# Quyans/GOI-Hyperplane

Measured on AMD Instinct MI355X. Metric: training views/sec (rasterizer fwd+bwd), 1M Gaussians @1600x1056 RGB+16-d feat, higher is better.
Workload: dtype f32

## Files before the change

### goi_hyperplane_amd/_lib.py

```python
from __future__ import annotations

import ctypes as C
import os

_HERE = os.path.dirname(os.path.abspath(__file__))
LIB_PATH = os.path.join(_HERE, "lib", "libgoi_raster.so")

ABI_VERSION = 8

STAGES = ("preprocess", "depth_sort", "scan", "emit", "tile_sort", "ranges", "blend_fwd", "blend_bwd",
          "preprocess_bwd")


class GoiRasterScene(C.Structure):
    _fields_ = [
        ("P", C.c_int), ("D", C.c_int), ("M", C.c_int), ("S", C.c_int), ("W", C.c_int), ("H", C.c_int),
        ("bg", C.c_void_p), ("means3D", C.c_void_p), ("shs", C.c_void_p), ("colors_precomp", C.c_void_p),
        ("semantics", C.c_void_p), ("opacities", C.c_void_p), ("scales", C.c_void_p),
        ("scale_modifier", C.c_float), ("rotations", C.c_void_p), ("cov3D_precomp", C.c_void_p),
        ("viewmatrix", C.c_void_p), ("projmatrix", C.c_void_p), ("campos", C.c_void_p),
        ("tan_fovx", C.c_float), ("tan_fovy", C.c_float), ("prefiltered", C.c_int), ("debug", C.c_int),
    ]


# ... 83 lines not shown
    "goi_raster_photometric_backward": (C.c_int, [C.c_void_p, C.c_void_p, C.c_longlong, C.c_int, C.c_int, C.c_int, C.c_int, C.c_float,
                                           C.c_uint] + [C.c_void_p] * 5),
    "goi_raster_densify_workspace_bytes": (C.c_size_t, [C.c_longlong]),
    "goi_raster_densify_stats": (C.c_int, [C.c_longlong, C.c_void_p, C.c_longlong] + [C.c_void_p] * 4),
    "goi_raster_densify_plan": (C.c_int, [C.c_longlong] + [C.c_void_p] * 4 + [C.c_double] * 3 + [C.c_int, C.c_double, C.c_double]
                                + [C.c_void_p] * 3),
    "goi_raster_densify_prune_plan": (C.c_int, [C.c_longlong] + [C.c_void_p] * 4),
    "goi_raster_densify_apply": (C.c_int, [C.c_longlong, C.c_void_p, C.c_int] + [C.c_void_p] * 3 + [C.c_longlong, C.c_longlong]
                                 + [C.c_void_p] * 2),
    "goi_raster_set_option": (C.c_int, [C.c_char_p, C.c_int]),
    "goi_raster_blend_stats": (C.c_int, [C.c_int] * 4 + [C.c_void_p] * 5),
    "goi_raster_debug_views": (C.c_int, [C.c_int] * 4 + [C.c_void_p] * 3 + [C.c_void_p] * 8 + [C.c_void_p]),
    "goi_raster_debug_sort_workspace_bytes": (C.c_size_t, [C.c_longlong, C.c_int, C.c_int]),
    "goi_raster_debug_sort_pairs": (C.c_int, [C.c_void_p] * 4 + [C.c_longlong, C.c_int, C.c_int, C.c_void_p, C.c_void_p, C.c_int]
                                    + [C.c_void_p] * 3),
    "goi_raster_debug_scan_workspace_bytes": (C.c_size_t, [C.c_longlong]),
    "goi_raster_debug_exclusive_scan": (C.c_int, [C.c_void_p] * 3 + [C.c_longlong] + [C.c_void_p] * 4),
    "goi_raster_debug_reduce_row_floats": (C.c_int, [C.c_int, C.c_int]),
    "goi_raster_debug_reduce_workspace_bytes": (C.c_size_t, [C.c_longlong]),
    "goi_raster_debug_reduce_rows": (C.c_int, [C.c_int, C.c_int, C.c_int, C.c_longlong] + [C.c_void_p] * 14),
    "goi_raster_debug_preprocess_backward": (C.c_int, [C.POINTER(GoiRasterScene), C.c_int, C.c_int, C.c_int, C.c_longlong]
                                             + [C.c_void_p] * 22),
    "goi_raster_debug_pair_eval": (C.c_int, [C.c_int, C.c_int, C.c_int, C.c_void_p, C.c_void_p, C.c_longlong] + [C.c_void_p] * 4),
    "goi_raster_debug_backward_blend": (C.c_int, [C.POINTER(GoiRasterScene), C.c_int, C.c_int] + [C.c_void_p] * 24),
}

_lib = None


def load():
# ... 69 lines not shown
```

### goi_hyperplane_amd/csrc/api.hip

```cpp
#include <climits>
#include <cmath>
#include <cstdio>
#include <cstring>
#include <cstdlib>
#include <atomic>
#include <chrono>
#include <mutex>
#include <thread>
#include <string>
#include <vector>

#include "common.h"

namespace goi {

namespace {

thread_local std::string g_err;

int fail(const char* where, hipError_t e) {
    g_err = std::string(where) + ": " + hipGetErrorString(e);
    return -1;
}
int fail(const std::string& msg) {
// ... 224 lines not shown
    GOI_HIP(hipMemsetAsync(g.blk_coarse, 0,
                           round_up_256((size_t)(reinterpret_cast<char*>(g.scratch + depth_ctrl) -
                                                 reinterpret_cast<char*>(g.blk_coarse))), s));
    {
        StageTimer t(GOI_STAGE_PREPROCESS, s);
        launch_preprocess_fwd(sc, g, radii, im.ranges, gx * gy, s, zcut, zlearn, keep, keep_invert);
    }
    if (check_stage(sc, s, "preprocess")) return -1;
    if (ticket >= 0 && enqueue_readback(g, ticket, s)) return -1;
    const bool onesweep = g_options.sort_variant == 1;
    const uint32_t* v_dev = g.counters + COUNTER_V;
    int order_idx;
    {
        StageTimer t(GOI_STAGE_DEPTH_SORT, s);
        launch_compact_listed(P, g, onesweep ? radix_sort_ghist(g.scratch, (size_t)P, 0, 32) : nullptr, !onesweep, s);
        order_idx = radix_sort_pairs(g.sort_keys, g.sort_vals, (size_t)P, 0, 32, g.scratch, s, true,
                                     onesweep, onesweep ? v_dev : nullptr, g.counters + COUNTER_SORTERR);
    }
    if (check_stage(sc, s, "depth sort")) return -1;
    *order_out = g.sort_vals[order_idx];
    {
        StageTimer t(GOI_STAGE_SCAN, s);
        exclusive_scan_u32(g.tiles_touched, *order_out, g.offsets, (size_t)P, nullptr, g.scratch, s, v_dev);
    }
    return 0;
}

int enqueue_back(const GoiRasterScene& sc, GeomView& g, ImageView& im, const BinView& bv_in, int cap, bool exact,
                 const uint32_t* order, const int* radii, const uint32_t** plist, hipStream_t s) {
    BinView bv = bv_in;
    const int P = sc.P;
    const int gx = (sc.W + TILE - 1) / TILE, gy = (sc.H + TILE - 1) / TILE;
// ... 5 lines not shown
        if (counting) {
            launch_emit_counting(P, sc.W, sc.H, g, order, radii, bv.keys[0], bv.vals[0], im.ranges, bv.scratch,
                                 radix_sort_control_words((size_t)cap, 0, tile_bits), (uint32_t)cap, s);
        }
        else if (cap > 0)
            launch_emit(P, sc.W, sc.H, g, order, radii, bv.keys[0], bv.vals[0], (uint32_t)cap, s);
    }
    if (check_stage(sc, s, "emit")) return -1;
    int fin;
    if (counting) {
        {
            StageTimer t(GOI_STAGE_RANGES, s);
            launch_tile_ranges_hist(sc.W, sc.H, im.ranges, radix_sort_ghist(bv.scratch, (size_t)cap, 0, tile_bits), g.counters, s);
        }
        StageTimer t(GOI_STAGE_TILE_SORT, s);
        fin = radix_sort_pairs(bv.keys, bv.vals, (size_t)cap, 0, tile_bits, bv.scratch, s, true,
                               true, n_dev, g.counters + COUNTER_OVF);
    } else {
        {
            StageTimer t(GOI_STAGE_TILE_SORT, s);
            fin = radix_sort_pairs(bv.keys, bv.vals, (size_t)cap, 0, tile_bits, bv.scratch, s, false, false, n_dev,
                                   g.counters + COUNTER_OVF);
        }
        if (check_stage(sc, s, "tile sort")) return -1;
        StageTimer t(GOI_STAGE_RANGES, s);
        launch_ranges(cap, n_dev, bv.keys[fin], im.ranges, gx * gy, s);
    }
    if (check_stage(sc, s, "tile sort / ranges")) return -1;
    *plist = bv.vals[fin];
    return 0;
}

// ... 980 lines not shown
int goi_raster_set_option(const char* name, int value) {
    if (!name) return fail("option name is NULL");
    std::lock_guard<std::mutex> lk(g_options_mu);
    Options& g_options = g_shared_options;
    if (!strcmp(name, "fwd_variant")) {
        if (value < 0 || value > 1) return fail("fwd_variant must be 0 or 1");
        g_options.fwd_variant = value;
    }
    else if (!strcmp(name, "bwd_variant")) {
        if (value < 0 || value > 2) return fail("bwd_variant must be 0, 1 or 2");
        g_options.bwd_variant = value;
    }
    else if (!strcmp(name, "sort_variant")) g_options.sort_variant = value;
    else if (!strcmp(name, "sort_small")) g_options.sort_small = value;
    else if (!strcmp(name, "sort_lookback")) g_options.sort_lookback = value;
    else if (!strcmp(name, "cull_variant")) g_options.cull_variant = value;
    else if (!strcmp(name, "bwd_order")) {
        if (value < 0 || value > 8) return fail("bwd_order must be 0 .. 8");
        g_options.bwd_order = value;
    }
    else if (!strcmp(name, "decode_variant")) g_options.decode_variant = value;
    else if (!strcmp(name, "bwd_masks")) {
        if (value < 0 || value > 1) return fail("bwd_masks must be 0 or 1");
        g_options.bwd_masks = value;
    }
    else if (!strcmp(name, "bwd_records")) {
        if (value < 0 || value > 2) return fail("bwd_records must be 0, 1 or 2");
        g_options.bwd_records = value;
    }
    else if (!strcmp(name, "bwd_skip_idle")) {
// ... 65 lines not shown
                                 hipMemcpyDeviceToDevice, s));
    }
    if (depths) GOI_HIP(hipMemcpy2DAsync(depths, 4, rec + 44, pitch, 4, P, hipMemcpyDeviceToDevice, s));
    if (rgb) GOI_HIP(hipMemcpy2DAsync(rgb, 12, rec + 32, pitch, 12, P, hipMemcpyDeviceToDevice, s));
    if (tiles_touched)
        GOI_HIP(hipMemcpyAsync(tiles_touched, g.tiles_touched, sizeof(uint32_t) * P, hipMemcpyDeviceToDevice, s));
    if (ranges) GOI_HIP(hipMemcpyAsync(ranges, im.ranges, sizeof(uint2) * gx * gy, hipMemcpyDeviceToDevice, s));
    if (n_contrib)
        GOI_HIP(hipMemcpyAsync(n_contrib, im.n_contrib, sizeof(uint32_t) * (size_t)W * H, hipMemcpyDeviceToDevice, s));
    if (point_list && R > 0) {
        BinView bv;
        binning_layout(R, const_cast<char*>(static_cast<const char*>(binning_buffer)), &bv);
        const int fin = tile_sort_result_index(W, H, R);
        GOI_HIP(hipMemcpyAsync(point_list, bv.vals[fin], sizeof(uint32_t) * (size_t)R, hipMemcpyDeviceToDevice, s));
    }
    return 0;
}

static int debug_sort_args(const char* fn, long long n, int lo, int hi) {
    if (n < 0 || n >= SORT_MAX_KEYS) return fail(std::string(fn) + ": need 0 <= n < 2^30");
    if (lo < 0 || hi > 32 || lo >= hi) return fail(std::string(fn) + ": need 0 <= lo < hi <= 32");
    return 0;
}

size_t goi_raster_debug_sort_workspace_bytes(long long n, int lo, int hi) {
    if (n < 0 || n >= SORT_MAX_KEYS || lo < 0 || hi > 32 || lo >= hi) return 0;
    return sort_scratch_words((size_t)(n > 0 ? n : 1)) * sizeof(uint32_t) + 256;
}

int goi_raster_debug_sort_pairs(uint32_t* keys0, uint32_t* vals0, uint32_t* keys1, uint32_t* vals1, long long n, int lo, int hi,
// ... 11 lines not shown
    const hipStream_t s = static_cast<hipStream_t>(stream);
    uint32_t* scratch = static_cast<uint32_t*>(workspace);
    bool cleared = (flags & 1) != 0;
    if (ghist) {
        const size_t passes = (size_t)(hi - lo + 7) / 8;
        GOI_HIP(hipMemsetAsync(scratch, 0, radix_sort_control_words((size_t)n, lo, hi) * sizeof(uint32_t), s));
        GOI_HIP(hipMemcpyAsync(radix_sort_ghist(scratch, (size_t)n, lo, hi), ghist, passes * 256 * sizeof(uint32_t),
                               hipMemcpyDeviceToDevice, s));
        cleared = true;
    }
    uint32_t* keys[2] = {keys0, keys1};
    uint32_t* vals[2] = {vals0, vals1};
    const int fin = radix_sort_pairs(keys, vals, (size_t)n, lo, hi, scratch, s, cleared, ghist != nullptr, n_dev, error_out);
    GOI_HIP(hipGetLastError());
    if (error_out) radix_sort_report_error(scratch, (size_t)n, lo, hi, error_out, s);
    GOI_HIP(hipGetLastError());
    return fin;
}

size_t goi_raster_debug_scan_workspace_bytes(long long n) {
    return (n >= 0 && n < (1ll << 32)) ? scan_scratch_words((size_t)n) * sizeof(uint32_t) + 256 : 0;
}

int goi_raster_debug_exclusive_scan(const uint32_t* in, const uint32_t* gather, uint32_t* out, long long n, const uint32_t* n_dev,
                                    uint32_t* total, void* workspace, void* stream) {
    refresh_options();
    if (n < 0 || n >= (1ll << 32)) return fail("goi_raster_debug_exclusive_scan: need 0 <= n < 2^32");
    if (gather && out == in) return fail("goi_raster_debug_exclusive_scan: out == in with a gather is a data race");
    const hipStream_t s = static_cast<hipStream_t>(stream);
    if (n > 0 && (!in || !out || !workspace)) return fail("goi_raster_debug_exclusive_scan: a required pointer is NULL");
// ... 251 lines not shown
```

### goi_hyperplane_amd/csrc/common.h

```cpp
#pragma once

#include <hip/hip_runtime.h>
#include <stddef.h>
#include <stdint.h>

#include "goi_raster.h"

namespace goi {

constexpr int TILE = 16;
constexpr int TILE_PIX = TILE * TILE;
constexpr int WAVE = 64;

struct GaussRec {
    float4 q0, q1, q2;
};

struct GeomView {
    GaussRec* rec;
    float* cov3D;
    uint32_t* tiles_touched;
    uint8_t* clamped;
    uint32_t* sort_keys[2];
    uint32_t* sort_vals[2];
// ... 47 lines not shown

__host__ __device__ inline unsigned long long* member_mask_ptr(unsigned long long* qmask0, unsigned long long* qmask, int tile,
                                                                int q, uint32_t x0, int r) {
    return r == 0 ? qmask0 + ((size_t)tile * 4 + q) : qmask + (((size_t)(x0 >> 6) + (size_t)r) * 4 + q);
}

size_t geom_layout(int P, char* base, GeomView* v);
size_t image_layout(int W, int H, char* base, ImageView* v);
size_t binning_layout(int N, char* base, BinView* v);

struct Options {
    int fwd_variant = 1;
    int bwd_variant = 0;
    int sort_variant = 1;
    int sort_lookback = 1;
    int sort_small = 0;
    int decode_variant = 1;
    int cull_variant = 2;
    int bwd_order = 1;
    int bwd_masks = 1;
    int bwd_records = 1;
    int bwd_skip_idle = 1;
    int osh_path = 0;
};
extern thread_local Options g_options;
void refresh_options();

size_t scan_scratch_words(size_t n);
size_t sort_scratch_words(size_t n);
void exclusive_scan_u32(const uint32_t* in, const uint32_t* gather, uint32_t* out, size_t n, uint32_t* total,
                        uint32_t* scratch, hipStream_t s, const uint32_t* n_dev = nullptr);
int radix_sort_pairs(uint32_t* keys[2], uint32_t* vals[2], size_t n, int lo, int hi, uint32_t* scratch,
                     hipStream_t s, bool cleared = false, bool ghist_ready = false, const uint32_t* n_dev = nullptr,
                     uint32_t* frame_error = nullptr);
size_t radix_sort_control_words(size_t n, int lo, int hi);
uint32_t* radix_sort_ghist(uint32_t* scratch, size_t n, int lo, int hi);
void radix_sort_report_error(const uint32_t* scratch, size_t n, int lo, int hi, uint32_t* out, hipStream_t s);
constexpr long long SORT_MAX_KEYS = 1ll << 30;

void launch_preprocess_fwd(const GoiRasterScene& sc, const GeomView& g, int* radii, uint2* ranges, int n_tiles,
                           hipStream_t s, const float* zcut = nullptr, uint32_t* zlearn = nullptr,
                           const uint8_t* keep = nullptr, int keep_invert = 0);
void launch_compact_listed(int P, const GeomView& g, uint32_t* ghist, bool pad, hipStream_t s);
constexpr int COARSE_BLOCKS = 32, COARSE_STRIDE = 8;
constexpr int SORT_MAX_PASSES = 4, SORT_GH_COPIES = 8;
constexpr int PRE_BLOCK = 256;
void launch_emit(int P, int W, int H, const GeomView& g, const uint32_t* order, const int* radii, uint32_t* keys,
                 uint32_t* vals, uint32_t cap, hipStream_t s);
bool emit_can_count_tiles(int W, int H);
// ... 179 lines not shown
constexpr int NR_STRIPES = 32, NR_STRIDE = 32, NR_BASE = 32;
constexpr int COUNTER_WORDS = NR_BASE + NR_STRIPES * NR_STRIDE;
constexpr int COUNTER_CULL = 2;
constexpr int COUNTER_N = 3;
constexpr int COUNTER_V = 5;
constexpr int COUNTER_OVF = 4;

constexpr uint32_t OVF_TRUNCATED = 1u, OVF_MISSORTED = 2u, OVF_CUT_TOO_TIGHT = 4u;
constexpr int COUNTER_BIGQ = 7;
constexpr int COUNTER_SORTERR = 6;

inline int depth_sort_result_index() { return ((32 + 7) / 8) & 1; }

inline int tile_key_bits(uint32_t n_tiles) { return n_tiles <= 1 ? 1 : 32 - __builtin_clz(n_tiles); }

}
```

### goi_hyperplane_amd/csrc/preprocess.hip

```cpp
#include <algorithm>
#include <type_traits>

#include "common.h"
#include "gmath.h"
#include "row_sum.h"

namespace goi {

namespace {

__device__ __forceinline__ float ndc_to_pix(float v, int S) { return (float)(((v + 1.0) * S - 1.0) * 0.5); }

__device__ __forceinline__ M3 rotation_from_quat(float r, float x, float y, float z) {
    return make_m3(1.f - 2.f * (y * y + z * z), 2.f * (x * y - r * z), 2.f * (x * z + r * y),
                   2.f * (x * y + r * z), 1.f - 2.f * (x * x + z * z), 2.f * (y * z - r * x),
                   2.f * (x * z - r * y), 2.f * (y * z + r * x), 1.f - 2.f * (x * x + y * y));
}

struct Cov2D {
    M3 T, Vrk, W;
    V3 t;
    float txtz, tytz, limx, limy;
    M3 cov;
};
// ... 222 lines not shown
                    for (int i = 0; i < 8; i++) {
                        const int bsafe = max(bits[i], 0);
                        zc[i] = a.zcut[(size_t)(y0 + bsafe / w) * a.gx + (x0 + bsafe % w)];
                    }
#pragma unroll
                    for (int i = 0; i < 8; i++)
                        if (bits[i] >= 0 && zc[i] < p_view.z) mask &= ~(1ull << bits[i]);
                }
            }
            tmask_v = mask;
            touched = (uint32_t)__popcll(mask);
        }
        key = __float_as_uint(p_view.z);
    }

    if (vis) {
        float4* r4 = reinterpret_cast<float4*>(rec + idx);
        r4[0] = make_float4(pix, piy, con_a, con_b);
        r4[1] = make_float4(con_c, o, hx, hy);
    }
    if (live) {
        radii[idx] = my_radius_i;
        tiles_touched[idx] = touched;
        raw_key[idx] = key;
        aux[idx] = make_uint4(0u, (uint32_t)my_radius_i, (uint32_t)tmask_v, (uint32_t)(tmask_v >> 32));
    }

    float cr = 0.f, cg = 0.f, cb = 0.f;
    V3 dir = {0.f, 0.f, 0.f};
    if (vis && !a.colors_precomp) {
        const V3 campos = {a.campos[0], a.campos[1], a.campos[2]};
        dir = p - campos;
        dir = dir / sqrtf(dot3(dir, dir));
    }
    auto finish_colour = [&](const V3& res) {
// ... 13 lines not shown
            if (row16) {
                const float4* r4 = reinterpret_cast<const float4*>(a.shs + (size_t)idx * 48);
#pragma unroll
                for (int i = 0; i < 12; i++) {
                    const float4 v = r4[i];
                    rowf[4 * i] = v.x;
                    rowf[4 * i + 1] = v.y;
                    rowf[4 * i + 2] = v.z;
                    rowf[4 * i + 3] = v.w;
                }
            }
            const V3* shg = reinterpret_cast<const V3*>(a.shs) + (size_t)idx * a.M;
            finish_colour(sh_to_rgb_sum(a.D, dir, [&](int k) { return row16 ? V3{rowf[3 * k], rowf[3 * k + 1], rowf[3 * k + 2]} : shg[k]; }));
        }
    }
    if (vis) reinterpret_cast<float4*>(rec + idx)[2] = make_float4(cr, cg, cb, p_view.z);
    if (live) clamped[idx] = clamp_bits;
    __shared__ uint32_t s_wsum[4], s_wvis[4];
    uint32_t wsum = live ? touched : 0u;
#pragma unroll
    for (int d = 32; d >= 1; d >>= 1) wsum += (uint32_t)__shfl_xor((int)wsum, d, 64);
    const uint32_t wvis = (uint32_t)__popcll(__ballot(live && touched > 0));
    if ((threadIdx.x & 63) == 0) {
        s_wsum[threadIdx.x >> 6] = wsum;
        s_wvis[threadIdx.x >> 6] = wvis;
    }
    __syncthreads();
    if (threadIdx.x == 0) {
        const uint32_t bsum = s_wsum[0] + s_wsum[1] + s_wsum[2] + s_wsum[3];
        if (bsum) atomicAdd(&counters[NR_BASE + NR_STRIDE * (blockIdx.x % NR_STRIPES)], bsum);
// ... 780 lines not shown
```

### goi_hyperplane_amd/csrc/scan_sort.hip

```cpp
#include <atomic>

#include "common.h"

namespace goi {

namespace {

constexpr int SCAN_THREADS = 256;
constexpr int SCAN_ITEMS = 8;
constexpr int SCAN_CHUNK = SCAN_THREADS * SCAN_ITEMS;

#ifndef GOI_SORT_THREADS
#define GOI_SORT_THREADS 512
#endif
constexpr int SORT_THREADS = GOI_SORT_THREADS;
constexpr int SORT_ITEMS = 16;
constexpr int SORT_TILE = SORT_THREADS * SORT_ITEMS;
constexpr int SORT_WAVES = SORT_THREADS / WAVE;
constexpr int SORT_WAVE_ITEMS = SORT_TILE / SORT_WAVES;
constexpr int RADIX_MAX = 256;

__device__ __forceinline__ uint32_t wave_inclusive_scan(uint32_t v, int lane) {
#pragma unroll
    for (int d = 1; d < WAVE; d <<= 1) {
// ... 237 lines not shown
            const uint32_t key = keys[i];
            for (int p = 0; p < plan.passes; p++)
                atomicAdd(&h[p][(key >> plan.shift[p]) & ((1u << plan.nbits[p]) - 1u)], 1u);
        }
    }
    __syncthreads();
    uint32_t* gh = ghist + (size_t)(blockIdx.x % SORT_GH_COPIES) * MAX_PASSES * RADIX_MAX;
    for (int i = threadIdx.x; i < plan.passes * RADIX_MAX; i += SORT_THREADS) {
        const uint32_t v = (&h[0][0])[i];
        if (v) atomicAdd(&gh[i], v);
    }
}

constexpr int SWEEP_TARGET_TILES = 512;
constexpr uint32_t SWEEP_GROUPED_MAX_TILES = 640;
template <int THREADS, int ITEMS>
__global__ __launch_bounds__(THREADS) void sweep_pass_k(const uint32_t* __restrict__ keys_in,
                                                             const uint32_t* __restrict__ vals_in,
                                                             uint32_t* __restrict__ keys_out,
                                                             uint32_t* __restrict__ vals_out, size_t n_cap,
                                                             const uint32_t* __restrict__ n_dev, int shift,
                                                             int nbits, const uint32_t* __restrict__ ghist,
                                                             uint32_t* status, uint32_t* ticket, uint32_t* error,
                                                             uint32_t* frame_error, int min_items, uint32_t* gstat) {
    constexpr int WAVES = THREADS / WAVE;
    __shared__ uint32_t cnt[WAVES][RADIX_MAX];
    __shared__ uint32_t gbase[RADIX_MAX];
    __shared__ uint32_t lbase[RADIX_MAX];
    __shared__ uint32_t s_gh[RADIX_MAX];
    extern __shared__ uint32_t s_dyn[];
    uint32_t* s_keys = s_dyn;
    uint32_t* s_vals = s_dyn + THREADS * ITEMS;
    __shared__ uint32_t s_bid;
    __shared__ uint32_t s_trivial;
    const uint32_t radix = 1u << nbits, mask = radix - 1u;
    const bool adaptive = min_items < ITEMS;
    uint32_t early_ticket = 0;
    if (!adaptive && threadIdx.x == 0) early_ticket = atomicAdd(ticket, 1u);
    uint32_t gh = 0;
    if (threadIdx.x < radix) {
#pragma unroll
        for (int c = 0; c < SORT_GH_COPIES; c++) gh += ghist[(size_t)c * MAX_PASSES * RADIX_MAX + threadIdx.x];
    }
    const size_t n = effective_n(n_cap, n_dev);
    int items = ITEMS;
    while (items > min_items && n <= (size_t)THREADS * (size_t)(items / 2) * SWEEP_TARGET_TILES) items >>= 1;
    const int TILE_KEYS = THREADS * items, WAVE_ITEMS = TILE_KEYS / WAVES;
    if (adaptive && (size_t)blockIdx.x * TILE_KEYS >= n) return;
    if (threadIdx.x == 0) s_trivial = 0u;
    for (int i = threadIdx.x; i < WAVES * RADIX_MAX; i += THREADS) (&cnt[0][0])[i] = 0;
    __syncthreads();
    if (threadIdx.x < RADIX_MAX) {
        s_gh[threadIdx.x] = gh;
        if (n > 0 && gh == (uint32_t)n) s_trivial = 1u;
    }
    if (threadIdx.x == 0) s_bid = adaptive ? atomicAdd(ticket, 1u) : early_ticket;
    __syncthreads();
    if (s_trivial) {
        const size_t base = (size_t)blockIdx.x * TILE_KEYS;
        for (int r = 0; r < items; r++) {
            const size_t i = base + (size_t)r * THREADS + threadIdx.x;
            if (i < n) {
                keys_out[i] = keys_in[i];
                vals_out[i] = vals_in[i];
            }
        }
        return;
    }
    const uint32_t bid = s_bid;
    if ((size_t)bid * TILE_KEYS >= n) return;
    const int lane = threadIdx.x & 63, w = threadIdx.x >> 6;
    const uint64_t lt = (1ull << lane) - 1ull;
    const size_t tile_base = (size_t)bid * TILE_KEYS;
    const size_t wbase = tile_base + (size_t)w * WAVE_ITEMS;
    uint32_t key[ITEMS], val[ITEMS], rank[ITEMS];
#pragma unroll
    for (int r = 0; r < ITEMS; r++) {
        size_t i = wbase + (size_t)r * WAVE + lane;
        const bool ok = r < items && i < n;
        key[r] = ok ? keys_in[i] : 0xFFFFFFFFu;
        val[r] = ok ? vals_in[i] : 0u;
    }
#pragma unroll
    for (int r = 0; r < ITEMS; r++) {
        if (r >= items) break;
        size_t i = wbase + (size_t)r * WAVE + lane;
        const bool ok = i < n;
        const uint32_t d = (key[r] >> shift) & mask;
        uint64_t peers = __ballot(ok);
#pragma unroll
        for (int b = 0; b < 8; b++) {
            if (b < nbits) {
                const bool bit = (d >> b) & 1u;
                const uint64_t bal = __ballot(bit);
                peers &= bit ? bal : ~bal;
            }
        }
        const uint32_t prev = ok ? cnt[w][d] : 0u;
        const uint32_t below = (uint32_t)__popcll(peers & lt);
        rank[r] = prev + below;
        __builtin_amdgcn_wave_barrier();
        if (ok && below == 0) cnt[w][d] = prev + (uint32_t)__popcll(peers);
        __builtin_amdgcn_wave_barrier();
// ... 110 lines not shown
        for (int k = 0; k < 4; k++) {
            const uint32_t d = threadIdx.x * 4 + k;
            if (d < radix) {
                gbase[d] += gr;
                lbase[d] = lr;
            }
            gr += g[k];
            lr += l[k];
        }
    }
    __syncthreads();
#pragma unroll
    for (int r = 0; r < ITEMS; r++) {
        size_t i = wbase + (size_t)r * WAVE + lane;
        if (r < items && i < n) {
            const uint32_t d = (key[r] >> shift) & mask;
            const uint32_t lp = lbase[d] + cnt[w][d] + rank[r];
            s_keys[lp] = key[r];
            s_vals[lp] = val[r];
        }
    }
    __syncthreads();
    const uint32_t count = (uint32_t)(tile_base + (size_t)TILE_KEYS <= n ? (size_t)TILE_KEYS : (n > tile_base ? n - tile_base : 0));
    for (uint32_t i = threadIdx.x; i < count; i += THREADS) {
        const uint32_t k = s_keys[i];
        const uint32_t d = (k >> shift) & mask;
        const uint32_t pos = gbase[d] + (i - lbase[d]);
        keys_out[pos] = k;
        vals_out[pos] = s_vals[i];
    }
}

inline size_t div_up(size_t a, size_t b) { return (a + b - 1) / b; }

}

size_t scan_scratch_words(size_t n) { return div_up(n, SCAN_CHUNK) + 16; }

static size_t sweep_group_rows(size_t tile_rows) { return tile_rows / 16 + 2; }
static int sweep_min_items_for(size_t n, bool small) {
    if (n <= ((size_t)2 << 20) && !small) return 4;
    int items = 2;
    while (items < 16 && (n + (size_t)512 * items - 1) / ((size_t)512 * items) > 2048) items <<= 1;
    return items;
// ... 37 lines not shown
}
uint32_t* radix_sort_ghist(uint32_t* scratch, size_t n, int lo, int hi) {
    return scratch + sweep_status_words(n, lo, hi);
}

namespace {
__global__ void or_word_k(const uint32_t* __restrict__ src, uint32_t* __restrict__ dst) { *dst |= *src; }
}

void radix_sort_report_error(const uint32_t* scratch, size_t n, int lo, int hi, uint32_t* out, hipStream_t s) {
    if (n == 0 || g_options.sort_variant != 1 || (hi - lo + 7) / 8 > MAX_PASSES) return;
    const uint32_t* error = scratch + sweep_status_words(n, lo, hi) + GH_WORDS + MAX_PASSES;
    or_word_k<<<dim3(1), dim3(1), 0, s>>>(error, out);
}

int radix_sort_pairs(uint32_t* keys[2], uint32_t* vals[2], size_t n, int lo, int hi, uint32_t* scratch,
                     hipStream_t s, bool cleared, bool ghist_ready, const uint32_t* n_dev, uint32_t* frame_error) {
    int cur = 0;
    if (n == 0) return cur;
    const uint32_t nblk = (uint32_t)div_up(n, SORT_TILE);
    uint32_t* table = scratch;
    uint32_t* scan_scratch = scratch + (size_t)RADIX_MAX * nblk;
    const int bits = hi - lo;
    const int passes = (bits + 7) / 8;
    int shift = lo;
    if (g_options.sort_variant == 1 && passes <= MAX_PASSES) {
        uint32_t* status = scratch;
        uint32_t* ghist = radix_sort_ghist(scratch, n, lo, hi);
        uint32_t* ticket = ghist + GH_WORDS;
        uint32_t* error = ticket + MAX_PASSES;
        if (!cleared) (void)hipMemsetAsync(status, 0, radix_sort_control_words(n, lo, hi) * sizeof(uint32_t), s);
        SweepPlan plan;
        plan.passes = passes;
        int sh = lo;
        for (int p = 0; p < passes; p++) {
            plan.nbits[p] = (bits - (sh - lo) + (passes - p) - 1) / (passes - p);
            plan.shift[p] = sh;
            sh += plan.nbits[p];
        }
        for (int p = passes; p < MAX_PASSES; p++) plan.shift[p] = plan.nbits[p] = 0;
        if (!ghist_ready) sweep_hist_k<<<dim3(nblk), dim3(SORT_THREADS), 0, s>>>(keys[0], n, n_dev, plan, ghist);
        const size_t tile = sweep_tile_keys(n);
        const int min_items = sweep_min_items(n);
        const uint32_t nt = (uint32_t)div_up(n, sweep_min_tile_keys(n));
        const size_t lds = 2 * tile * sizeof(uint32_t);
        static std::atomic<uint64_t> attr_set{0};
        int dev_id = 0;
        (void)hipGetDevice(&dev_id);
        const uint64_t dev_bit = 1ull << (dev_id & 63);
        if (!(attr_set.load(std::memory_order_relaxed) & dev_bit)) {
            (void)hipFuncSetAttribute(reinterpret_cast<const void*>(sweep_pass_k<512, 16>),
                                      hipFuncAttributeMaxDynamicSharedMemorySize, 2 * 8192 * (int)sizeof(uint32_t));
            attr_set.fetch_or(dev_bit, std::memory_order_relaxed);
        }
        const size_t prow = (size_t)nt + sweep_group_rows(nt);
        for (int p = 0; p < passes; p++) {
            uint32_t* st_p = status + (size_t)p * prow * RADIX_MAX;
            uint32_t* gst_p = g_options.sort_lookback ? st_p + (size_t)nt * RADIX_MAX : nullptr;
            if (tile == 4096)
                sweep_pass_k<1024, 4><<<dim3(nt), dim3(1024), lds, s>>>(
                    keys[cur], vals[cur], keys[cur ^ 1], vals[cur ^ 1], n, n_dev, plan.shift[p], plan.nbits[p],
                    ghist + (size_t)p * RADIX_MAX, st_p, ticket + p, error, frame_error, 4, gst_p);
            else
                sweep_pass_k<512, 16><<<dim3(nt), dim3(512), lds, s>>>(
                    keys[cur], vals[cur], keys[cur ^ 1], vals[cur ^ 1], n, n_dev, plan.shift[p], plan.nbits[p],
                    ghist + (size_t)p * RADIX_MAX, st_p, ticket + p, error, frame_error, min_items, gst_p);
            cur ^= 1;
        }
        return cur;
    }
    for (int p = 0; p < passes; p++) {
        const int nbits = (bits - (shift - lo) + (passes - p) - 1) / (passes - p);
        const uint32_t mask = (1u << nbits) - 1u;
        radix_hist_k<<<dim3(nblk), dim3(SORT_THREADS), 0, s>>>(keys[cur], n, shift, mask, table, nblk);
        const size_t tab_n = (size_t)(mask + 1u) * nblk;
        exclusive_scan_u32(table, nullptr, table, tab_n, nullptr, scan_scratch, s);
        radix_scatter_k<<<dim3(nblk), dim3(SORT_THREADS), 0, s>>>(keys[cur], vals[cur], keys[cur ^ 1], vals[cur ^ 1], n,
                                                                  shift, nbits, table, nblk);
        cur ^= 1;
        shift += nbits;
    }
    return cur;
}

}
```

### include/goi_raster.h

```cpp
#ifndef GOI_RASTER_H
#define GOI_RASTER_H

#include <stddef.h>
#include <stdint.h>

#ifdef __cplusplus
extern "C" {
#endif

#define GOI_RASTER_ABI_VERSION 8

typedef struct GoiRasterScene {
    int P;
    int D;
    int M;
    int S;
    int W, H;
    const float* bg;
    const float* means3D;
    const float* shs;
    const float* colors_precomp;
    const float* semantics;
    const float* opacities;
    const float* scales;
// ... 247 lines not shown
                            double big_threshold, unsigned* counts, void* workspace, void* stream);
int goi_raster_densify_prune_plan(long long P, const unsigned char* mask, unsigned* counts, void* workspace, void* stream);
int goi_raster_densify_apply(long long P, const GoiDensifyRows* groups, int n_groups, const float* rotation, const float* scaling,
                             const float* z, long long n_split, long long kept_children, const void* workspace, void* stream);

#define GOI_BLEND_STATS_WORDS 16
int goi_raster_blend_stats(int P, int W, int H, int R, const void* geom_buffer, const void* binning_buffer,
                           const void* image_buffer, unsigned long long* counters, void* stream);

int goi_raster_debug_views(int P, int W, int H, int R, const void* geom_buffer, const void* binning_buffer,
                           const void* image_buffer,
                           float* depths , float* means2D , float* conic_opacity ,
                           float* rgb , uint32_t* tiles_touched , uint32_t* point_list ,
                           uint32_t* ranges , uint32_t* n_contrib , void* stream);

size_t goi_raster_debug_sort_workspace_bytes(long long n, int lo, int hi);
int goi_raster_debug_sort_pairs(uint32_t* keys0, uint32_t* vals0, uint32_t* keys1, uint32_t* vals1, long long n, int lo, int hi,
                                const uint32_t* n_dev, const uint32_t* ghist, int flags, uint32_t* error_out, void* workspace,
                                void* stream);
size_t goi_raster_debug_scan_workspace_bytes(long long n);
int goi_raster_debug_exclusive_scan(const uint32_t* in, const uint32_t* gather, uint32_t* out, long long n, const uint32_t* n_dev,
                                    uint32_t* total, void* workspace, void* stream);

int goi_raster_debug_reduce_row_floats(int mode, int S);
size_t goi_raster_debug_reduce_workspace_bytes(long long n_cap);
int goi_raster_debug_reduce_rows(int mode, int P, int S, long long n_cap, const uint32_t* frame, const uint32_t* order,
                                 const uint32_t* offsets, const uint32_t* tiles_touched, float* rows, const uint8_t* flags,
                                 float* dL_dmean2D, float* dL_dconic, float* dL_dopacity, float* dL_dcolor, float* dL_dsemantic,
                                 float* dL_ddepth, void* workspace, void* stream);

int goi_raster_debug_preprocess_backward(const GoiRasterScene* scene, int source, int flags, int max_blocks, long long n_cap,
                                         const uint32_t* frame, const int* radii, const uint8_t* clamped, const float* cov3D,
                                         const int* prev_radii, const uint32_t* aux, const uint32_t* tiles_touched,
                                         const float* rows, const uint8_t* row_flags, float* dL_dmean2D, const float* dL_dconic,
// ... 20 lines not shown
```

Before: 804.8.

## Skip key writes in final sort pass and pack high digit into values

Adds radix_sort_vals, which drops the key output on the last onesweep pass, since only the value order is consumed. For two-pass tile sorts where P fits, the first pass also packs the next pass's digit into the high bits of the value word, so the second pass reads no keys. This cuts global key reads and writes and shrinks LDS use in the depth and tile sorts. The risk is that correctness depends on the P bound check, and extra template variants increase code size. Debug entry points and a preprocess store-placement macro are also added.

```diff
diff --git a/goi_hyperplane_amd/_lib.py b/goi_hyperplane_amd/_lib.py
--- a/goi_hyperplane_amd/_lib.py
+++ b/goi_hyperplane_amd/_lib.py
@@ -121,6 +121,10 @@
     "goi_raster_debug_sort_workspace_bytes": (C.c_size_t, [C.c_longlong, C.c_int, C.c_int]),
     "goi_raster_debug_sort_pairs": (C.c_int, [C.c_void_p] * 4 + [C.c_longlong, C.c_int, C.c_int, C.c_void_p, C.c_void_p, C.c_int]
                                     + [C.c_void_p] * 3),
+    "goi_raster_debug_depth_order": (C.c_int, [C.c_int] + [C.c_void_p] * 4),
+    "goi_raster_tile_sort_plan": (C.c_int, [C.c_longlong, C.c_longlong]),
+    "goi_raster_debug_tile_sort": (C.c_int, [C.c_void_p] * 4 + [C.c_longlong, C.c_void_p, C.c_longlong, C.c_longlong]
+                                   + [C.c_void_p] * 3),
     "goi_raster_debug_scan_workspace_bytes": (C.c_size_t, [C.c_longlong]),
     "goi_raster_debug_exclusive_scan": (C.c_int, [C.c_void_p] * 3 + [C.c_longlong] + [C.c_void_p] * 4),
     "goi_raster_debug_reduce_row_floats": (C.c_int, [C.c_int, C.c_int]),
diff --git a/goi_hyperplane_amd/csrc/api.hip b/goi_hyperplane_amd/csrc/api.hip
--- a/goi_hyperplane_amd/csrc/api.hip
+++ b/goi_hyperplane_amd/csrc/api.hip
@@ -262,8 +262,8 @@
     {
         StageTimer t(GOI_STAGE_DEPTH_SORT, s);
         launch_compact_listed(P, g, onesweep ? radix_sort_ghist(g.scratch, (size_t)P, 0, 32) : nullptr, !onesweep, s);
-        order_idx = radix_sort_pairs(g.sort_keys, g.sort_vals, (size_t)P, 0, 32, g.scratch, s, true,
-                                     onesweep, onesweep ? v_dev : nullptr, g.counters + COUNTER_SORTERR);
+        order_idx = radix_sort_vals(g.sort_keys, g.sort_vals, (size_t)P, 0, 32, SORT_VALS_NOKEYS, g.scratch, s, true,
+                                    onesweep, onesweep ? v_dev : nullptr, g.counters + COUNTER_SORTERR);
     }
     if (check_stage(sc, s, "depth sort")) return -1;
     *order_out = g.sort_vals[order_idx];
@@ -299,8 +299,8 @@
             launch_tile_ranges_hist(sc.W, sc.H, im.ranges, radix_sort_ghist(bv.scratch, (size_t)cap, 0, tile_bits), g.counters, s);
         }
         StageTimer t(GOI_STAGE_TILE_SORT, s);
-        fin = radix_sort_pairs(bv.keys, bv.vals, (size_t)cap, 0, tile_bits, bv.scratch, s, true,
-                               true, n_dev, g.counters + COUNTER_OVF);
+        fin = radix_sort_vals(bv.keys, bv.vals, (size_t)cap, 0, tile_bits, tile_sort_plan((uint32_t)(gx * gy), (uint64_t)P), bv.scratch,
+                              s, true, true, n_dev, g.counters + COUNTER_OVF);
     } else {
         {
             StageTimer t(GOI_STAGE_TILE_SORT, s);
@@ -1311,6 +1311,10 @@
     else if (!strcmp(name, "sort_variant")) g_options.sort_variant = value;
     else if (!strcmp(name, "sort_small")) g_options.sort_small = value;
     else if (!strcmp(name, "sort_lookback")) g_options.sort_lookback = value;
+    else if (!strcmp(name, "sort_pack")) {
+        if (value < 0 || value > 1) return fail("sort_pack must be 0 or 1");
+        g_options.sort_pack = value;
+    }
     else if (!strcmp(name, "cull_variant")) g_options.cull_variant = value;
     else if (!strcmp(name, "bwd_order")) {
         if (value < 0 || value > 8) return fail("bwd_order must be 0 .. 8");
@@ -1406,6 +1410,18 @@
         const int fin = tile_sort_result_index(W, H, R);
         GOI_HIP(hipMemcpyAsync(point_list, bv.vals[fin], sizeof(uint32_t) * (size_t)R, hipMemcpyDeviceToDevice, s));
     }
+    return 0;
+}
+
+int goi_raster_debug_depth_order(int P, const void* geom_buffer, uint32_t* order, uint32_t* offsets, void* stream) {
+    hipStream_t s = static_cast<hipStream_t>(stream);
+    if (P <= 0) return 0;
+    if (!geom_buffer) return fail("goi_raster_debug_depth_order: workspace pointer is NULL");
+    GeomView g;
+    geom_layout(P, const_cast<char*>(static_cast<const char*>(geom_buffer)), &g);
+    if (order)
+        GOI_HIP(hipMemcpyAsync(order, g.sort_vals[depth_sort_result_index()], sizeof(uint32_t) * P, hipMemcpyDeviceToDevice, s));
+    if (offsets) GOI_HIP(hipMemcpyAsync(offsets, g.offsets, sizeof(uint32_t) * P, hipMemcpyDeviceToDevice, s));
     return 0;
 }
 
@@ -1447,6 +1463,35 @@
     const int fin = radix_sort_pairs(keys, vals, (size_t)n, lo, hi, scratch, s, cleared, ghist != nullptr, n_dev, error_out);
     GOI_HIP(hipGetLastError());
     if (error_out) radix_sort_report_error(scratch, (size_t)n, lo, hi, error_out, s);
+    GOI_HIP(hipGetLastError());
+    return fin;
+}
+
+int goi_raster_tile_sort_plan(long long n_tiles, long long P) {
+    if (n_tiles < 1 || n_tiles > 0x7FFFFFFFll || P < 0) return fail("goi_raster_tile_sort_plan: need 1 <= n_tiles < 2^31 and P >= 0");
+    return tile_sort_plan((uint32_t)n_tiles, (uint64_t)P);
+}
+
+int goi_raster_debug_tile_sort(uint32_t* keys0, uint32_t* vals0, uint32_t* keys1, uint32_t* vals1, long long n, const uint32_t* n_dev,
+                               long long n_tiles, long long P, uint32_t* error_out, void* workspace, void* stream) {
+    refresh_options();
+    const char* fn = "goi_raster_debug_tile_sort";
+    if (n < 0 || n >= SORT_MAX_KEYS) return fail(std::string(fn) + ": need 0 <= n < 2^30");
+    if (n_tiles < 1 || n_tiles > 65535) return fail(std::string(fn) + ": need 1 <= n_tiles < 2^16 (the counting path's key width)");
+    if (P < 1 || P > (1ll << 32)) return fail(std::string(fn) + ": need 1 <= P <= 2^32");
+    if (g_options.sort_variant != 1) return fail(std::string(fn) + ": needs the onesweep sort (sort_variant 1)");
+    if (n == 0) return 0;
+    if (!keys0 || !vals0 || !keys1 || !vals1 || !workspace) return fail(std::string(fn) + ": a required pointer is NULL");
+    if (reinterpret_cast<uintptr_t>(workspace) & 255) return fail(std::string(fn) + ": workspace must be 256-byte aligned");
+    const hipStream_t s = static_cast<hipStream_t>(stream);
+    uint32_t* scratch = static_cast<uint32_t*>(workspace);
+    const int tile_bits = tile_key_bits((uint32_t)n_tiles);
+    uint32_t* keys[2] = {keys0, keys1};
+    uint32_t* vals[2] = {vals0, vals1};
+    const int fin = radix_sort_vals(keys, vals, (size_t)n, 0, tile_bits, tile_sort_plan((uint32_t)n_tiles, (uint64_t)P), scratch, s,
+                                    false, false, n_dev, error_out);
+    GOI_HIP(hipGetLastError());
+    if (error_out) radix_sort_report_error(scratch, (size_t)n, 0, tile_bits, error_out, s);
     GOI_HIP(hipGetLastError());
     return fin;
 }
diff --git a/goi_hyperplane_amd/csrc/common.h b/goi_hyperplane_amd/csrc/common.h
--- a/goi_hyperplane_amd/csrc/common.h
+++ b/goi_hyperplane_amd/csrc/common.h
@@ -85,6 +85,7 @@
     int bwd_variant = 0;
     int sort_variant = 1;
     int sort_lookback = 1;
+    int sort_pack = 1;
     int sort_small = 0;
     int decode_variant = 1;
     int cull_variant = 2;
@@ -104,6 +105,10 @@
 int radix_sort_pairs(uint32_t* keys[2], uint32_t* vals[2], size_t n, int lo, int hi, uint32_t* scratch,
                      hipStream_t s, bool cleared = false, bool ghist_ready = false, const uint32_t* n_dev = nullptr,
                      uint32_t* frame_error = nullptr);
+enum { SORT_VALS_PLAIN = 0, SORT_VALS_NOKEYS = 1, SORT_VALS_PACKED = 2 };
+int radix_sort_vals(uint32_t* keys[2], uint32_t* vals[2], size_t n, int lo, int hi, int plan, uint32_t* scratch,
+                    hipStream_t s, bool cleared = false, bool ghist_ready = false, const uint32_t* n_dev = nullptr,
+                    uint32_t* frame_error = nullptr);
 size_t radix_sort_control_words(size_t n, int lo, int hi);
 uint32_t* radix_sort_ghist(uint32_t* scratch, size_t n, int lo, int hi);
 void radix_sort_report_error(const uint32_t* scratch, size_t n, int lo, int hi, uint32_t* out, hipStream_t s);
@@ -313,4 +318,13 @@
 
 inline int tile_key_bits(uint32_t n_tiles) { return n_tiles <= 1 ? 1 : 32 - __builtin_clz(n_tiles); }
 
-}
+inline int tile_sort_plan(uint32_t n_tiles, uint64_t P) {
+    const int bits = tile_key_bits(n_tiles);
+    const int passes = (bits + 7) / 8;
+    if (passes == 1) return SORT_VALS_NOKEYS;
+    if (passes != 2) return SORT_VALS_PLAIN;
+    const int n0 = (bits + passes - 1) / passes, n1 = bits - n0;
+    return P <= (1ull << (32 - n1)) ? SORT_VALS_PACKED : SORT_VALS_PLAIN;
+}
+
+}
diff --git a/goi_hyperplane_amd/csrc/preprocess.hip b/goi_hyperplane_amd/csrc/preprocess.hip
--- a/goi_hyperplane_amd/csrc/preprocess.hip
+++ b/goi_hyperplane_amd/csrc/preprocess.hip
@@ -260,11 +260,13 @@
         key = __float_as_uint(p_view.z);
     }
 
+#ifndef GOI_PRE_SINGLE_STORE
     if (vis) {
         float4* r4 = reinterpret_cast<float4*>(rec + idx);
         r4[0] = make_float4(pix, piy, con_a, con_b);
         r4[1] = make_float4(con_c, o, hx, hy);
     }
+#endif
     if (live) {
         radii[idx] = my_radius_i;
         tiles_touched[idx] = touched;
@@ -308,6 +310,13 @@
             finish_colour(sh_to_rgb_sum(a.D, dir, [&](int k) { return row16 ? V3{rowf[3 * k], rowf[3 * k + 1], rowf[3 * k + 2]} : shg[k]; }));
         }
     }
+#ifdef GOI_PRE_SINGLE_STORE
+    if (vis) {
+        float4* r4 = reinterpret_cast<float4*>(rec + idx);
+        r4[0] = make_float4(pix, piy, con_a, con_b);
+        r4[1] = make_float4(con_c, o, hx, hy);
+    }
+#endif
     if (vis) reinterpret_cast<float4*>(rec + idx)[2] = make_float4(cr, cg, cb, p_view.z);
     if (live) clamped[idx] = clamp_bits;
     __shared__ uint32_t s_wsum[4], s_wvis[4];
diff --git a/goi_hyperplane_amd/csrc/scan_sort.hip b/goi_hyperplane_amd/csrc/scan_sort.hip
--- a/goi_hyperplane_amd/csrc/scan_sort.hip
+++ b/goi_hyperplane_amd/csrc/scan_sort.hip
@@ -275,7 +275,8 @@
 
 constexpr int SWEEP_TARGET_TILES = 512;
 constexpr uint32_t SWEEP_GROUPED_MAX_TILES = 640;
-template <int THREADS, int ITEMS>
+enum { SWEEP_PAIRS = 0, SWEEP_NOKEYS = 1, SWEEP_PACK_OUT = 2, SWEEP_PACK_IN = 3 };
+template <int THREADS, int ITEMS, int MODE = SWEEP_PAIRS>
 __global__ __launch_bounds__(THREADS) void sweep_pass_k(const uint32_t* __restrict__ keys_in,
                                                              const uint32_t* __restrict__ vals_in,
                                                              uint32_t* __restrict__ keys_out,
@@ -283,15 +284,26 @@
                                                              const uint32_t* __restrict__ n_dev, int shift,
                                                              int nbits, const uint32_t* __restrict__ ghist,
                                                              uint32_t* status, uint32_t* ticket, uint32_t* error,
-                                                             uint32_t* frame_error, int min_items, uint32_t* gstat) {
+                                                             uint32_t* frame_error, int min_items, uint32_t* gstat,
+                                                             int pack_bits) {
     constexpr int WAVES = THREADS / WAVE;
+    constexpr bool KEYS_IN = MODE != SWEEP_PACK_IN, KEYS_OUT = MODE == SWEEP_PAIRS;
+    constexpr bool BYTE_DIGITS = MODE == SWEEP_NOKEYS || MODE == SWEEP_PACK_OUT;
     __shared__ uint32_t cnt[WAVES][RADIX_MAX];
     __shared__ uint32_t gbase[RADIX_MAX];
     __shared__ uint32_t lbase[RADIX_MAX];
     __shared__ uint32_t s_gh[RADIX_MAX];
     extern __shared__ uint32_t s_dyn[];
     uint32_t* s_keys = s_dyn;
-    uint32_t* s_vals = s_dyn + THREADS * ITEMS;
+    uint32_t* s_vals = KEYS_OUT ? s_dyn + THREADS * ITEMS : s_dyn;
+    uint8_t* s_dig = reinterpret_cast<uint8_t*>(s_dyn + THREADS * ITEMS);
+    const uint32_t pack_shift = MODE == SWEEP_PACK_IN ? 32u - (uint32_t)nbits : MODE == SWEEP_PACK_OUT ? 32u - (uint32_t)pack_bits : 0u;
+    const uint32_t pack_mask = MODE == SWEEP_PACK_OUT ? (1u << pack_bits) - 1u : 0u;
+    auto out_word = [&](uint32_t k, uint32_t v) -> uint32_t {
+        if (MODE == SWEEP_PACK_OUT) return v | (((k >> (shift + nbits)) & pack_mask) << pack_shift);
+        if (MODE == SWEEP_PACK_IN) return v & ((1u << pack_shift) - 1u);
+        return v;
+    };
     __shared__ uint32_t s_bid;
     __shared__ uint32_t s_trivial;
     const uint32_t radix = 1u << nbits, mask = radix - 1u;
@@ -322,8 +334,8 @@
         for (int r = 0; r < items; r++) {
             const size_t i = base + (size_t)r * THREADS + threadIdx.x;
             if (i < n) {
-                keys_out[i] = keys_in[i];
-                vals_out[i] = vals_in[i];
+                if (KEYS_OUT) keys_out[i] = keys_in[i];
+                vals_out[i] = out_word(MODE == SWEEP_PACK_OUT ? keys_in[i] : 0u, vals_in[i]);
             }
         }
         return;
@@ -339,15 +351,17 @@
     for (int r = 0; r < ITEMS; r++) {
         size_t i = wbase + (size_t)r * WAVE + lane;
         const bool ok = r < items && i < n;
-        key[r] = ok ? keys_in[i] : 0xFFFFFFFFu;
         val[r] = ok ? vals_in[i] : 0u;
-    }
+        if (KEYS_IN) key[r] = ok ? keys_in[i] : 0xFFFFFFFFu;
+        else key[r] = val[r] >> pack_shift;
+    }
+    auto digit = [&](uint32_t k) -> uint32_t { return KEYS_IN ? (k >> shift) & mask : k; };
 #pragma unroll
     for (int r = 0; r < ITEMS; r++) {
         if (r >= items) break;
         size_t i = wbase + (size_t)r * WAVE + lane;
         const bool ok = i < n;
-        const uint32_t d = (key[r] >> shift) & mask;
+        const uint32_t d = digit(key[r]);
         uint64_t peers = __ballot(ok);
 #pragma unroll
         for (int b = 0; b < 8; b++) {
@@ -488,20 +502,22 @@
     for (int r = 0; r < ITEMS; r++) {
         size_t i = wbase + (size_t)r * WAVE + lane;
         if (r < items && i < n) {
-            const uint32_t d = (key[r] >> shift) & mask;
+            const uint32_t d = digit(key[r]);
             const uint32_t lp = lbase[d] + cnt[w][d] + rank[r];
-            s_keys[lp] = key[r];
-            s_vals[lp] = val[r];
+            if (KEYS_OUT) s_keys[lp] = key[r];
+            if (BYTE_DIGITS) s_dig[lp] = (uint8_t)d;
+            s_vals[lp] = MODE == SWEEP_PACK_OUT ? out_word(key[r], val[r]) : val[r];
         }
     }
     __syncthreads();
     const uint32_t count = (uint32_t)(tile_base + (size_t)TILE_KEYS <= n ? (size_t)TILE_KEYS : (n > tile_base ? n - tile_base : 0));
     for (uint32_t i = threadIdx.x; i < count; i += THREADS) {
-        const uint32_t k = s_keys[i];
-        const uint32_t d = (k >> shift) & mask;
+        const uint32_t v = s_vals[i];
+        const uint32_t k = KEYS_OUT ? s_keys[i] : 0u;
+        const uint32_t d = KEYS_OUT ? (k >> shift) & mask : BYTE_DIGITS ? (uint32_t)s_dig[i] : v >> pack_shift;
         const uint32_t pos = gbase[d] + (i - lbase[d]);
-        keys_out[pos] = k;
-        vals_out[pos] = s_vals[i];
+        if (KEYS_OUT) keys_out[pos] = k;
+        vals_out[pos] = MODE == SWEEP_PACK_IN ? out_word(0u, v) : v;
     }
 }
 
@@ -569,8 +585,27 @@
     or_word_k<<<dim3(1), dim3(1), 0, s>>>(error, out);
 }
 
-int radix_sort_pairs(uint32_t* keys[2], uint32_t* vals[2], size_t n, int lo, int hi, uint32_t* scratch,
-                     hipStream_t s, bool cleared, bool ghist_ready, const uint32_t* n_dev, uint32_t* frame_error) {
+namespace {
+template <int MODE>
+void launch_sweep_pass(size_t tile, uint32_t nt, hipStream_t s, const uint32_t* keys_in, const uint32_t* vals_in, uint32_t* keys_out,
+                       uint32_t* vals_out, size_t n, const uint32_t* n_dev, int shift, int nbits, const uint32_t* ghist,
+                       uint32_t* status, uint32_t* ticket, uint32_t* error, uint32_t* frame_error, int min_items, uint32_t* gstat,
+                       int pack_bits) {
+    const size_t lds = MODE == SWEEP_PAIRS ? 2 * tile * sizeof(uint32_t)
+                                           : MODE == SWEEP_PACK_IN ? tile * sizeof(uint32_t) : tile * (sizeof(uint32_t) + 1);
+#define GOI_SWEEP_ARGS keys_in, vals_in, keys_out, vals_out, n, n_dev, shift, nbits, ghist, status, ticket, error, frame_error
+    if constexpr (MODE == SWEEP_PAIRS) {
+        if (tile == 4096) sweep_pass_k<1024, 4><<<dim3(nt), dim3(1024), lds, s>>>(GOI_SWEEP_ARGS, 4, gstat, 0);
+        else sweep_pass_k<512, 16><<<dim3(nt), dim3(512), lds, s>>>(GOI_SWEEP_ARGS, min_items, gstat, 0);
+    } else {
+        if (tile == 4096) sweep_pass_k<1024, 4, MODE><<<dim3(nt), dim3(1024), lds, s>>>(GOI_SWEEP_ARGS, 4, gstat, pack_bits);
+        else sweep_pass_k<512, 16, MODE><<<dim3(nt), dim3(512), lds, s>>>(GOI_SWEEP_ARGS, min_items, gstat, pack_bits);
+    }
+#undef GOI_SWEEP_ARGS
+}
+
+int radix_sort_impl(uint32_t* keys[2], uint32_t* vals[2], size_t n, int lo, int hi, uint32_t* scratch, hipStream_t s, bool cleared,
+                    bool ghist_ready, const uint32_t* n_dev, uint32_t* frame_error, int vals_plan) {
     int cur = 0;
     if (n == 0) return cur;
     const uint32_t nblk = (uint32_t)div_up(n, SORT_TILE);
@@ -598,7 +633,6 @@
         const size_t tile = sweep_tile_keys(n);
         const int min_items = sweep_min_items(n);
         const uint32_t nt = (uint32_t)div_up(n, sweep_min_tile_keys(n));
-        const size_t lds = 2 * tile * sizeof(uint32_t);
         static std::atomic<uint64_t> attr_set{0};
         int dev_id = 0;
         (void)hipGetDevice(&dev_id);
@@ -609,17 +643,21 @@
             attr_set.fetch_or(dev_bit, std::memory_order_relaxed);
         }
         const size_t prow = (size_t)nt + sweep_group_rows(nt);
+        const bool packed = vals_plan == SORT_VALS_PACKED && passes == 2;
         for (int p = 0; p < passes; p++) {
             uint32_t* st_p = status + (size_t)p * prow * RADIX_MAX;
             uint32_t* gst_p = g_options.sort_lookback ? st_p + (size_t)nt * RADIX_MAX : nullptr;
-            if (tile == 4096)
-                sweep_pass_k<1024, 4><<<dim3(nt), dim3(1024), lds, s>>>(
-                    keys[cur], vals[cur], keys[cur ^ 1], vals[cur ^ 1], n, n_dev, plan.shift[p], plan.nbits[p],
-                    ghist + (size_t)p * RADIX_MAX, st_p, ticket + p, error, frame_error, 4, gst_p);
-            else
-                sweep_pass_k<512, 16><<<dim3(nt), dim3(512), lds, s>>>(
-                    keys[cur], vals[cur], keys[cur ^ 1], vals[cur ^ 1], n, n_dev, plan.shift[p], plan.nbits[p],
-                    ghist + (size_t)p * RADIX_MAX, st_p, ticket + p, error, frame_error, min_items, gst_p);
+            const int mode = packed ? (p == 0 ? SWEEP_PACK_OUT : SWEEP_PACK_IN)
+                             : vals_plan != SORT_VALS_PLAIN && p == passes - 1 ? SWEEP_NOKEYS : SWEEP_PAIRS;
+            const int pack_bits = mode == SWEEP_PACK_OUT ? plan.nbits[1] : 0;
+#define GOI_SWEEP_PASS(M)                                                                                                      \
+    launch_sweep_pass<M>(tile, nt, s, keys[cur], vals[cur], keys[cur ^ 1], vals[cur ^ 1], n, n_dev, plan.shift[p], plan.nbits[p], \
+                         ghist + (size_t)p * RADIX_MAX, st_p, ticket + p, error, frame_error, min_items, gst_p, pack_bits)
+            if (mode == SWEEP_PACK_OUT) GOI_SWEEP_PASS(SWEEP_PACK_OUT);
+            else if (mode == SWEEP_PACK_IN) GOI_SWEEP_PASS(SWEEP_PACK_IN);
+            else if (mode == SWEEP_NOKEYS) GOI_SWEEP_PASS(SWEEP_NOKEYS);
+            else GOI_SWEEP_PASS(SWEEP_PAIRS);
+#undef GOI_SWEEP_PASS
             cur ^= 1;
         }
         return cur;
@@ -637,5 +675,17 @@
     }
     return cur;
 }
-
-}
+}
+
+int radix_sort_pairs(uint32_t* keys[2], uint32_t* vals[2], size_t n, int lo, int hi, uint32_t* scratch,
+                     hipStream_t s, bool cleared, bool ghist_ready, const uint32_t* n_dev, uint32_t* frame_error) {
+    return radix_sort_impl(keys, vals, n, lo, hi, scratch, s, cleared, ghist_ready, n_dev, frame_error, SORT_VALS_PLAIN);
+}
+
+int radix_sort_vals(uint32_t* keys[2], uint32_t* vals[2], size_t n, int lo, int hi, int plan, uint32_t* scratch,
+                    hipStream_t s, bool cleared, bool ghist_ready, const uint32_t* n_dev, uint32_t* frame_error) {
+    return radix_sort_impl(keys, vals, n, lo, hi, scratch, s, cleared, ghist_ready, n_dev, frame_error,
+                           g_options.sort_pack ? plan : SORT_VALS_PLAIN);
+}
+
+}
diff --git a/include/goi_raster.h b/include/goi_raster.h
--- a/include/goi_raster.h
+++ b/include/goi_raster.h
@@ -285,10 +285,15 @@
                            float* rgb , uint32_t* tiles_touched , uint32_t* point_list ,
                            uint32_t* ranges , uint32_t* n_contrib , void* stream);
 
+int goi_raster_debug_depth_order(int P, const void* geom_buffer, uint32_t* order, uint32_t* offsets, void* stream);
+
 size_t goi_raster_debug_sort_workspace_bytes(long long n, int lo, int hi);
 int goi_raster_debug_sort_pairs(uint32_t* keys0, uint32_t* vals0, uint32_t* keys1, uint32_t* vals1, long long n, int lo, int hi,
                                 const uint32_t* n_dev, const uint32_t* ghist, int flags, uint32_t* error_out, void* workspace,
                                 void* stream);
+int goi_raster_tile_sort_plan(long long n_tiles, long long P);
+int goi_raster_debug_tile_sort(uint32_t* keys0, uint32_t* vals0, uint32_t* keys1, uint32_t* vals1, long long n, const uint32_t* n_dev,
+                               long long n_tiles, long long P, uint32_t* error_out, void* workspace, void* stream);
 size_t goi_raster_debug_scan_workspace_bytes(long long n);
 int goi_raster_debug_exclusive_scan(const uint32_t* in, const uint32_t* gather, uint32_t* out, long long n, const uint32_t* n_dev,
                                     uint32_t* total, void* workspace, void* stream);
```

Result: no change. 809.8, median of 5 (+0.6%).
